# cristianpjensen/thesis-pai-reconstruction

Measured on AMD Instinct MI355X. Metric: train images/sec (256x256, bs=64) Pix2Pix step, higher is better.
Workload: dtype bf16; 1 GPU; Pix2Pix generator+PatchGAN GAN step, 256x256x1 pairs, 64 images/GPU (BASELINE configs[1]); global_batch=64, per_gpu_batch=64, loss_type=gan, parallelism=dp1, grad_bucket_dtype=f32

## Files before the change

### thesis-pai-reconstruction_amd/csrc/gg_thin.hip

```cpp
#include <stdlib.h>

#include "common.h"

#ifndef THIN_ABL
#define THIN_ABL 0
#endif
typedef __attribute__((ext_vector_type(8))) __bf16 bf8_t;
typedef __attribute__((ext_vector_type(4))) __bf16 bf4_t;
typedef __attribute__((ext_vector_type(4))) float f4_t;
typedef __attribute__((ext_vector_type(8))) short s8_t;
typedef __attribute__((ext_vector_type(8))) unsigned short us8_t;

__device__ uint4 g_zero_line_thin[16];


__device__ __forceinline__ bf8_t relu8(bf8_t f) {
    s8_t x = __builtin_bit_cast(s8_t, f);
    const s8_t z = {0, 0, 0, 0, 0, 0, 0, 0};
    return __builtin_bit_cast(bf8_t, __builtin_elementwise_max(x, z));
}

template <int S>
__device__ __forceinline__ us8_t thin_gather8(__amdgpu_buffer_rsrc_t rs, int e0, int ix0, int TW, bool valid) {
    typedef __attribute__((ext_vector_type(4))) unsigned u4_t;
    const int base = ix0 & ~1, o = ix0 & 1;
    const bool neg = valid && e0 + base < 0;
    const unsigned vo = valid ? (neg ? 0u : (unsigned)(e0 + base) * 2u) : 0x80000000u;
    unsigned out[4];
    if (S == 2) {
        u4_t a = __builtin_amdgcn_raw_buffer_load_b128(rs, (int)vo, 0, 0);
        u4_t b = __builtin_amdgcn_raw_buffer_load_b128(rs, (int)vo + 16, 0, 0);
        if (__builtin_amdgcn_ballot_w64(neg) != 0) {
            if (neg) { b = (u4_t){a[3], b[0], b[1], b[2]}; a = (u4_t){0u, a[0], a[1], a[2]}; }
        }
        const unsigned sel = o ? 0x07060302u : 0x05040100u;
        out[0] = __builtin_amdgcn_perm(a[1], a[0], sel);
        out[1] = __builtin_amdgcn_perm(a[3], a[2], sel);
        out[2] = __builtin_amdgcn_perm(b[1], b[0], sel);
        out[3] = __builtin_amdgcn_perm(b[3], b[2], sel);
    } else {
        u4_t a = __builtin_amdgcn_raw_buffer_load_b128(rs, (int)vo, 0, 0);
        unsigned a4 = __builtin_amdgcn_raw_buffer_load_b32(rs, (int)vo + 16, 0, 0);
        if (__builtin_amdgcn_ballot_w64(neg) != 0) {
            if (neg) { a4 = a[3]; a = (u4_t){0u, a[0], a[1], a[2]}; }
        }
        const unsigned sh = (unsigned)o * 16u;
        out[0] = __builtin_amdgcn_alignbit(a[1], a[0], sh);
        out[1] = __builtin_amdgcn_alignbit(a[2], a[1], sh);
        out[2] = __builtin_amdgcn_alignbit(a[3], a[2], sh);
        out[3] = __builtin_amdgcn_alignbit(a4, a[3], sh);
    }
    const bool edge = valid && (ix0 < 0 || ix0 + S * 7 >= TW);
    if (__builtin_amdgcn_ballot_w64(edge) != 0) {
// ... 160 lines not shown
    int p0 = (blockIdx.x * 4 + wid) * 16;
    us8_t pv = {0, 0, 0, 0, 0, 0, 0, 0};
    if (p0 < g.M) pv = fast ? gather_fast(p0) : gather(p0);
    for (; p0 < g.M; p0 += pstep) {
        const int m = p0 + fr;
        us8_t pnext = {0, 0, 0, 0, 0, 0, 0, 0};
        if (p0 + pstep < g.M) pnext = fast ? gather_fast(p0 + pstep) : gather(p0 + pstep);
        const bf8_t bfrag = __builtin_bit_cast(bf8_t, pv);
#pragma unroll
        for (int gq = 0; gq < 2; ++gq) {
            if (gq * 4 >= mtiles) break;
            float v[16];
#pragma unroll
            for (int q = 0; q < 4; ++q) {
                f4_t acc = {0.f, 0.f, 0.f, 0.f};
                acc = __builtin_amdgcn_mfma_f32_16x16x32_bf16(af[gq * 4 + q], bfrag, acc, 0, 0, 0);
#pragma unroll
                for (int r = 0; r < 4; ++r) v[4 * q + r] = acc[r] + bias[gq][4 * q + r];
            }
            if (m >= g.M) continue;
            if ((THIN_ABL & 2) && v[0] != 12345.f) continue;
            const int co = 64 * gq + (sect ? 8 : 16) * fq;
            const int hop = sect ? 32 : 8;
            const size_t pix = (size_t)m;
            if (a.y1 || a.y2) {
                unsigned pk[8];
#pragma unroll
                for (int e = 0; e < 8; ++e) pk[e] = pk2bf(v[2 * e], v[2 * e + 1]);
                bf16_t* dst = (co < g.D1) ? (bf16_t*)a.y1 + pix * g.D1 + co : (bf16_t*)a.y2 + pix * g.D2 + (co - g.D1);
                *(uint4*)dst = make_uint4(pk[0], pk[1], pk[2], pk[3]);
                *(uint4*)(dst + hop) = make_uint4(pk[4], pk[5], pk[6], pk[7]);
            }
            if (a.yact) {
                unsigned pk[8];
#pragma unroll
                for (int e = 0; e < 8; ++e) {
                    float v0 = fmaxf(v[2 * e], act_slope * v[2 * e]), v1 = fmaxf(v[2 * e + 1], act_slope * v[2 * e + 1]);
                    v0 = v0 < act_floor ? act_floor : v0;
                    v1 = v1 < act_floor ? act_floor : v1;
                    pk[e] = pk2bf(v0, v1);
                }
                bf16_t* dst = (bf16_t*)a.yact + pix * g.Cout + co;
                *(uint4*)dst = make_uint4(pk[0], pk[1], pk[2], pk[3]);
                *(uint4*)(dst + hop) = make_uint4(pk[4], pk[5], pk[6], pk[7]);
            }
        }
        pv = pnext;
    }
}

#ifndef THIN_BWD_WAVES
#define THIN_BWD_WAVES 1
#endif
template <int T, bool RAW, int ACTM, int NG, bool BWD = false>
__global__ __launch_bounds__(256, BWD ? THIN_BWD_WAVES : 1) void thin_fwd2_k(GG g, FwdArgs a) {
    const int tid = threadIdx.x, lane = tid & 63, wid = tid >> 6;
    const int fr = lane & 15, fq = lane >> 4;
    const bf16_t* w = (const bf16_t*)a.w;
    constexpr int mtiles = 4 * NG;
    constexpr int KT = 16 * T;
    bf8_t af[4 * NG];
#pragma unroll
    for (int mt = 0; mt < 4 * NG; ++mt) {
        us8_t z = {0, 0, 0, 0, 0, 0, 0, 0};
        const int co = 64 * (mt >> 2) + 32 * ((mt & 3) >> 1) + 8 * (fr >> 2) + 4 * (mt & 1) + (fr & 3);
        if (mt < mtiles && 8 * fq < KT) z = *(const us8_t*)(w + (size_t)co * KT + 8 * fq);
        af[mt] = __builtin_bit_cast(bf8_t, z);
    }
    f4_t bias4[NG][4];
#pragma unroll
    for (int gq = 0; gq < NG; ++gq)
#pragma unroll
        for (int q = 0; q < 4; ++q)
#pragma unroll
            for (int r = 0; r < 4; ++r)
                bias4[gq][q][r] = (!BWD && a.bias) ? a.bias[64 * gq + 32 * (q >> 1) + 8 * fq + 4 * (q & 1) + r] : 0.f;
    const int pdx0 = g.dx[0][(8 * fq < KT) ? (8 * fq) / T : 0];
    const int pdyA = g.dy[0][(8 * fq < KT) ? (8 * fq) / T : 0];
    const int pdyB = g.dy[0][(8 * fq + 4 < KT) ? (8 * fq + 4) / T : 0];
    const unsigned thin_bytes = (unsigned)(g.N * g.H * g.W) * 2u;
    const __amdgpu_buffer_rsrc_t rs1 = __builtin_amdgcn_make_buffer_rsrc(const_cast<void*>(a.x1), 0, thin_bytes, 0x00020000);
    const __amdgpu_buffer_rsrc_t rs2 = __builtin_amdgcn_make_buffer_rsrc(const_cast<void*>(T == 2 ? a.x2 : a.x1), 0, thin_bytes, 0x00020000);
    const bool lane_k = 8 * fq < KT;
    auto gather_fast = [&](int p0) {
        const int m = p0 + fr;
        int n, gy, gx;
        decode_row2(g, m < g.M ? m : 0, n, gy, gx);
        const int ix0 = gx * g.S + pdx0;
        const int iyA = gy * g.S + pdyA, iyB = gy * g.S + pdyB;
        const bool okA = lane_k && m < g.M && (unsigned)iyA < (unsigned)g.H;
        uint2 pa, pb;
        if (T == 1) {
            const bool okB = lane_k && m < g.M && (unsigned)iyB < (unsigned)g.H;
            pa = thin_gather4(rs1, (n * g.H + iyA) * g.W, ix0, g.W, okA);
            pb = thin_gather4(rs1, (n * g.H + iyB) * g.W, ix0, g.W, okB);
            if (g.relu1) { pa.x = relu2u(pa.x); pa.y = relu2u(pa.y); pb.x = relu2u(pb.x); pb.y = relu2u(pb.y); }
        } else {
            uint2 qa = thin_gather4(rs1, (n * g.H + iyA) * g.W, ix0, g.W, okA);
            uint2 qb = thin_gather4(rs2, (n * g.H + iyA) * g.W, ix0, g.W, okA);
            if (g.relu1) { qa.x = relu2u(qa.x); qa.y = relu2u(qa.y); }
            if (g.relu2) { qb.x = relu2u(qb.x); qb.y = relu2u(qb.y); }
            pa = make_uint2(__builtin_amdgcn_perm(qb.x, qa.x, 0x05040100u), __builtin_amdgcn_perm(qb.x, qa.x, 0x07060302u));
            pb = make_uint2(__builtin_amdgcn_perm(qb.y, qa.y, 0x05040100u), __builtin_amdgcn_perm(qb.y, qa.y, 0x07060302u));
        }
        return __builtin_bit_cast(us8_t, make_uint4(pa.x, pa.y, pb.x, pb.y));
    };
    const unsigned raw1_bytes = (unsigned)g.M * (unsigned)g.D1 * 2u, raw2_bytes = (unsigned)g.M * (unsigned)g.D2 * 2u;
    const __amdgpu_buffer_rsrc_t y1rs = __builtin_amdgcn_make_buffer_rsrc(a.y1, 0, RAW ? raw1_bytes : 0u, 0x00020000);
// ... 16 lines not shown
    us8_t pq[AHEAD];
#pragma unroll
    for (int i = 0; i < AHEAD; ++i) {
        pq[i] = (us8_t){0, 0, 0, 0, 0, 0, 0, 0};
        if ((int64_t)p0 + (int64_t)i * pstep < g.M) pq[i] = gather_fast(p0 + i * pstep);
    }
#ifndef THIN_ZA
#define THIN_ZA 2
#endif
    constexpr int ZA = THIN_ZA;
    u4_t zql[BWD ? ZA : 1], zqh[BWD ? ZA : 1];
    if (BWD) {
#pragma unroll
        for (int i = 0; i < ZA; ++i) {
            zql[i] = __builtin_amdgcn_raw_buffer_load_b128(zrs, (int)(o_r1 + (unsigned)i * s_r1), 0, 0);
            zqh[i] = __builtin_amdgcn_raw_buffer_load_b128(zrs, (int)(o_r1 + (unsigned)i * s_r1) + 64, 0, 0);
        }
    }
    for (; p0 < g.M; p0 += pstep) {
        us8_t pnext = {0, 0, 0, 0, 0, 0, 0, 0};
        if ((int64_t)p0 + (int64_t)AHEAD * pstep < g.M) pnext = gather_fast(p0 + AHEAD * pstep);
        const bf8_t bfrag = __builtin_bit_cast(bf8_t, pq[0]);
        u4_t zlo = {0u, 0u, 0u, 0u}, zhi = {0u, 0u, 0u, 0u};
        if (BWD) {
            zlo = zql[0]; zhi = zqh[0];
#pragma unroll
            for (int i = 0; i + 1 < ZA; ++i) { zql[i] = zql[i + 1]; zqh[i] = zqh[i + 1]; }
            const unsigned long long zo = (unsigned long long)o_r1 + (unsigned long long)ZA * s_r1;
            const int zoff = zo < (unsigned long long)raw1_bytes ? (int)(unsigned)zo : (int)0x80000000u;
            zql[ZA - 1] = __builtin_amdgcn_raw_buffer_load_b128(zrs, zoff, 0, 0);
            zqh[ZA - 1] = __builtin_amdgcn_raw_buffer_load_b128(zrs, zoff + 64, 0, 0);
        }
#pragma unroll
        for (int gq = 0; gq < NG; ++gq) {
            f4_t acc[4];
#pragma unroll
            for (int q = 0; q < 4; ++q) acc[q] = __builtin_amdgcn_mfma_f32_16x16x32_bf16(af[gq * 4 + q], bfrag, bias4[gq][q], 0, 0, 0);
            if (RAW) {
                const u4_t lo = {pk2bf(acc[0][0], acc[0][1]), pk2bf(acc[0][2], acc[0][3]), pk2bf(acc[1][0], acc[1][1]), pk2bf(acc[1][2], acc[1][3])};
                const u4_t hi = {pk2bf(acc[2][0], acc[2][1]), pk2bf(acc[2][2], acc[2][3]), pk2bf(acc[3][0], acc[3][1]), pk2bf(acc[3][2], acc[3][3])};
                if (BWD && gq == 0 && p0 + fr < g.M) {
#pragma unroll
                    for (int e = 0; e < 4; ++e) {
                        const float g0 = __uint_as_float(lo[e] << 16), g1 = __uint_as_float(lo[e] & 0xffff0000u);
                        const float h0 = __uint_as_float(hi[e] << 16), h1 = __uint_as_float(hi[e] & 0xffff0000u);
                        bs1[2 * e] += g0; bs1[2 * e + 1] += g1; bs1[8 + 2 * e] += h0; bs1[8 + 2 * e + 1] += h1;
                        bs2[2 * e] = fmaf(g0, __uint_as_float(zlo[e] << 16), bs2[2 * e]);
                        bs2[2 * e + 1] = fmaf(g1, __uint_as_float(zlo[e] & 0xffff0000u), bs2[2 * e + 1]);
                        bs2[8 + 2 * e] = fmaf(h0, __uint_as_float(zhi[e] << 16), bs2[8 + 2 * e]);
                        bs2[8 + 2 * e + 1] = fmaf(h1, __uint_as_float(zhi[e] & 0xffff0000u), bs2[8 + 2 * e + 1]);
                    }
                }
                if (gq == 1 && second_raw) {
                    __builtin_amdgcn_raw_buffer_store_b128(lo, y2rs, (int)o_r2, 0, 0);
                    __builtin_amdgcn_raw_buffer_store_b128(hi, y2rs, (int)o_r2 + 64, 0, 0);
                } else {
                    __builtin_amdgcn_raw_buffer_store_b128(lo, y1rs, (int)o_r1 + 128 * gq, 0, 0);
                    __builtin_amdgcn_raw_buffer_store_b128(hi, y1rs, (int)o_r1 + 128 * gq + 64, 0, 0);
                }
            }
            if (ACTM) {
#pragma unroll
                for (int q = 0; q < 4; ++q)
#pragma unroll
                    for (int r = 0; r < 4; ++r) {
                        if (ACTM == 1) acc[q][r] = fmaxf(acc[q][r], 0.2f * acc[q][r]);
                        else if (ACTM == 2) acc[q][r] = acc[q][r] < 0.f ? 0.f : acc[q][r];
                    }
                const u4_t lo = {pk2bf(acc[0][0], acc[0][1]), pk2bf(acc[0][2], acc[0][3]), pk2bf(acc[1][0], acc[1][1]), pk2bf(acc[1][2], acc[1][3])};
                const u4_t hi = {pk2bf(acc[2][0], acc[2][1]), pk2bf(acc[2][2], acc[2][3]), pk2bf(acc[3][0], acc[3][1]), pk2bf(acc[3][2], acc[3][3])};
                __builtin_amdgcn_raw_buffer_store_b128(lo, yars, (int)o_act + 128 * gq, 0, 0);
                __builtin_amdgcn_raw_buffer_store_b128(hi, yars, (int)o_act + 128 * gq + 64, 0, 0);
            }
        }
        o_act += s_act; o_r1 += s_r1; o_r2 += s_r2;
#pragma unroll
        for (int i = 0; i + 1 < AHEAD; ++i) pq[i] = pq[i + 1];
        pq[AHEAD - 1] = pnext;
    }
    if (BWD) {
        __shared__ float red[4][2][64];
#pragma unroll
        for (int c = 0; c < 16; ++c) {
            float s1 = bs1[c], s2 = bs2[c];
            s1 += __builtin_bit_cast(float, __builtin_amdgcn_update_dpp(0, __builtin_bit_cast(int, s1), 0xB1, 0xF, 0xF, false));
            s2 += __builtin_bit_cast(float, __builtin_amdgcn_update_dpp(0, __builtin_bit_cast(int, s2), 0xB1, 0xF, 0xF, false));
            s1 += __builtin_bit_cast(float, __builtin_amdgcn_update_dpp(0, __builtin_bit_cast(int, s1), 0x4E, 0xF, 0xF, false));
            s2 += __builtin_bit_cast(float, __builtin_amdgcn_update_dpp(0, __builtin_bit_cast(int, s2), 0x4E, 0xF, 0xF, false));
            s1 += __builtin_bit_cast(float, __builtin_amdgcn_update_dpp(0, __builtin_bit_cast(int, s1), 0x141, 0xF, 0xF, false));
            s2 += __builtin_bit_cast(float, __builtin_amdgcn_update_dpp(0, __builtin_bit_cast(int, s2), 0x141, 0xF, 0xF, false));
            s1 += __builtin_bit_cast(float, __builtin_amdgcn_update_dpp(0, __builtin_bit_cast(int, s1), 0x140, 0xF, 0xF, false));
            s2 += __builtin_bit_cast(float, __builtin_amdgcn_update_dpp(0, __builtin_bit_cast(int, s2), 0x140, 0xF, 0xF, false));
            if (fr == 0) {
                const int ch = (c < 8) ? 8 * fq + c : 32 + 8 * fq + (c - 8);
                red[wid][0][ch] = s1;
                red[wid][1][ch] = s2;
            }
        }
        __syncthreads();
        if (tid < 64) {
            const float s1 = red[0][0][tid] + red[1][0][tid] + red[2][0][tid] + red[3][0][tid];
            const float s2 = red[0][1][tid] + red[1][1][tid] + red[2][1][tid] + red[3][1][tid];
            float* row = a.bpart + (size_t)blockIdx.x * 2 * g.D1;
            row[tid] = s1;
            row[g.D1 + tid] = a.brstd[tid] * (s2 - a.bmean[tid] * s1);
        }
    }
}

template <int T>
static void launch_thin_fwd2(const GG& g, const FwdArgs& a, int blocks, hipStream_t s) {
    const bool raw = a.y1 || a.y2;
    const int actm = !a.yact ? 0 : (a.eact == PAI_ACT_LRELU ? 1 : (a.eact == PAI_ACT_RELU ? 2 : 3));
#define TF2(RAWV, ACTV)                                                                                   \
    do {                                                                                                  \
        if (g.Cout == 64) PAI_LAUNCH((thin_fwd2_k<T, RAWV, ACTV, 1>), dim3(blocks), dim3(256), 0, s, g, a); \
        else PAI_LAUNCH((thin_fwd2_k<T, RAWV, ACTV, 2>), dim3(blocks), dim3(256), 0, s, g, a);             \
    } while (0)
    if (raw && a.bz) {
        PAI_LAUNCH((thin_fwd2_k<1, true, 0, 2, true>), dim3(blocks), dim3(256), 0, s, g, a);
    } else if (raw) {
        if (actm == 0) TF2(true, 0); else if (actm == 1) TF2(true, 1); else if (actm == 2) TF2(true, 2); else TF2(true, 3);
    } else {
        if (actm == 1) TF2(false, 1); else if (actm == 2) TF2(false, 2); else TF2(false, 3);
    }
#undef TF2
}

static int thin_fwd_blocks(const GG& g) {
    int blocks = cdiv(g.M, 64);
    static const int cap = getenv("PAI_TF_BLOCKS") ? atoi(getenv("PAI_TF_BLOCKS")) : 4096;
    return blocks > cap ? cap : blocks;
}

static bool thin_fwd2_ok(const GG& g, const FwdArgs& a) {
    const bool fast = pai_tunable("thin_fast", 1) && (g.W % 2) == 0 && (int64_t)g.N * g.H * g.W * 2 < (1ll << 31) &&
                      pai_tunable("thin_sect", 1) && (g.D2 == 0 || (g.D1 % 64) == 0);
    const bool out_ok = (a.y1 || a.y2 || a.yact) && (!a.yact || a.eact != PAI_ACT_TANH) && (!a.y2 || a.y1) &&
                        (int64_t)g.M * g.Cout * 2 < (1ll << 32) && (g.D2 == 0 || (g.D1 == 64 && g.D2 == 64));
    return pai_tunable("thin_fwd2", 1) && fast && g.ntaps == 16 && out_ok && (g.Cout == 64 || g.Cout == 128) &&
           !(a.yact && (a.y1 || a.y2) && g.D2 > 0);
}

int thin_fwd_bwd_rows(int dtype, const GG& g, const FwdArgs& a, int act1, const void* add, const float* scale) {
    if (!thin_fwd_ok(dtype, g, a) || !thin_fwd2_ok(g, a) || !pai_tunable("thin_bwd", 1)) return 0;
    if (g.C2 != 0 || g.D1 != 64 || g.D2 != 64 || !a.y1 || !a.y2 || a.yact || act1 != PAI_ACT_NONE || add || scale) return 0;
    return thin_fwd_blocks(g);
}

int launch_thin_fwd(const GG& g, const FwdArgs& a, hipStream_t s) {
    int blocks = thin_fwd_blocks(g);
    int fast_ok = pai_tunable("thin_fast", 1) && (g.W % 2) == 0 && (int64_t)g.N * g.H * g.W * 2 < (1ll << 31);
    if (pai_tunable("thin_sect", 1) && (g.D2 == 0 || (g.D1 % 64) == 0)) fast_ok |= 2;
    if (thin_fwd2_ok(g, a)) {
        if (g.C2 == 0) launch_thin_fwd2<1>(g, a, blocks, s);
        else launch_thin_fwd2<2>(g, a, blocks, s);
        PAI_LAUNCH_CHECK();
        return 0;
    }
    if (g.C2 == 0) PAI_LAUNCH(thin_fwd_k<1>, dim3(blocks), dim3(256), 0, s, g, a, fast_ok);
    else PAI_LAUNCH(thin_fwd_k<2>, dim3(blocks), dim3(256), 0, s, g, a, fast_ok);
    PAI_LAUNCH_CHECK();
    return 0;
}

bool head_dgrad_ok(int dtype, const GG& g, const FwdArgs& a) {
    return dtype == PAI_BF16 && pai_tunable("head_dgrad", 1) && g.nphase == 1 && g.ntaps == 16 && g.S == 1 && g.OS == 1 &&
           g.C1 == 1 && g.C2 == 0 && g.D2 == 0 && g.Cout == g.D1 && (g.Cout % 8) == 0 && g.Cout <= 1024 && g.OW <= 64 &&
           g.H * g.W <= 4096 && a.y1 && !a.y2 && !a.yact && !a.yf32 && !a.stats && !a.bias && !g.relu1 && !a.badd &&
           !a.bscale && !a.bpart && !a.skip_d1;
}

__global__ __launch_bounds__(256) void head_dgrad_k(GG g, FwdArgs a) {
    extern __shared__ __attribute__((aligned(16))) unsigned char hsm[];
    bf16_t* wt = (bf16_t*)hsm;
    float* src = (float*)(hsm + (size_t)16 * g.Cout * 2);
    const int tid = threadIdx.x;
    const int n = blockIdx.x / g.OH, oy = blockIdx.x - n * g.OH;
    const bf16_t* w = (const bf16_t*)a.w;
    for (int i = tid; i < g.Cout * 16; i += 256) {
        const int c = i >> 4, t = i & 15;
        wt[t * g.Cout + c] = w[i];
    }
    const bf16_t* x = (const bf16_t*)a.x1 + (size_t)n * g.H * g.W;
// ... 260 lines not shown
        else if (T == 1) PAI_LAUNCH((thin_up_k<1, 2>), grid, dim3(256), 0, s, g, a, t0, tx, ty);
        else if (g.Cin == 128) PAI_LAUNCH((thin_up_k<2, 4>), grid, dim3(256), 0, s, g, a, t0, tx, ty);
        else PAI_LAUNCH((thin_up_k<2, 2>), grid, dim3(256), 0, s, g, a, t0, tx, ty);
        PAI_LAUNCH_CHECK();
        return 0;
    }
    int blocks = cdiv((int64_t)g.N * g.H * g.W, 256);
    if (blocks > 4096) blocks = 4096;
#define TDG(TT, KK) PAI_LAUNCH((thin_dgrad_gemm_k<TT, KK>), dim3(blocks), dim3(256), 0, s, g, a, pai_ctx()->scratch, t0)
#define TDG_K(TT)                                     \
    switch (g.Cin / 32) {                             \
        case 1: TDG(TT, 1); break;                    \
        case 2: TDG(TT, 2); break;                    \
        case 4: TDG(TT, 4); break;                    \
        case 8: TDG(TT, 8); break;                    \
        case 16: TDG(TT, 16); break;                  \
        default: PAI_CHECK(false, "thin dgrad: unsupported Cin %d", g.Cin); \
    }
    if (T == 1) { TDG_K(1) } else { TDG_K(2) }
#undef TDG_K
#undef TDG
    PAI_LAUNCH_CHECK();
    PAI_CHECK((int64_t)g.N * g.OH * g.OW < (1ll << 31), "thin dgrad: more than 2^31 output pixels");
    int64_t b2 = ((int64_t)g.N * g.OH * g.OW + 255) / 256;
    if (b2 > 8192) b2 = 8192;
    PAI_LAUNCH(thin_col2im_k, dim3((int)b2), dim3(256), 0, s, g, a, (const float*)pai_ctx()->scratch, T, t0);
    PAI_LAUNCH_CHECK();
    return 0;
}

struct ThinW {
    const bf16_t *thin1, *thin2;
    const bf16_t *wide1, *wide2;
    int N, H, W, TH, TW, WC1, WC2;
    int relu1, relu2;
    int lw, lh;
    int tmul, flip;
    int kw, ntaps;
    float* dw;
    int s_wc, s_tap, s_t;
    float* dbias;
    int M;
    int fast;
    int pair;
    float* partial;
};

__device__ __forceinline__ int tw_swz(int row) { return ((row & 3) << 2) | ((row >> 2) & 3); }
__device__ __forceinline__ unsigned tw_off(int row, int ch) { return (unsigned)(256 * row + 16 * (ch ^ tw_swz(row))); }

#ifndef THIN_WG_WAVES
#define THIN_WG_WAVES 1
#endif
template <int T>
__global__ __launch_bounds__(256, THIN_WG_WAVES) void thin_wgrad_k(ThinW p, int chunks_per_block) {
    extern __shared__ __attribute__((aligned(16))) unsigned char smem[];
    const int tid = threadIdx.x, lane = tid & 63;
    const int wid = __builtin_amdgcn_readfirstlane(tid >> 6);
    const int fr = lane & 15, fq = lane >> 4, tq = fr >> 2, tp = fr & 3;
    const int wc0 = blockIdx.y * 128;
    const int WC = min(p.WC1 + p.WC2 - wc0, 128);
    const int pair = p.pair;
    const int ntile = pair ? 8 : WC / 16;
    const int ks = wid & 1;
    const int nt0 = (wid >> 1) * (ntile / 2);
    const int ntn = ntile / 2;
    const int pixh = pair ? (wid >> 1) * 64 : 0;
    const int CH = pair ? 128 : 64;
    const bf16_t* zero = (const bf16_t*)g_zero_line_thin;

    const int sc = lane & 15, sr = wid * 4 + (lane >> 4);
    const int gch = sc ^ tw_swz(sr);
    const bf16_t* wsrc;
    int wstride, wcol;
    bool wvalid = pair || gch * 8 < WC;
    const int wpix = pair ? (gch >> 3) * 64 : 0;
    if (pair) { wsrc = p.wide1; wstride = p.WC1; wcol = (gch & 7) * 8; }
    else if (wc0 + gch * 8 < p.WC1) { wsrc = p.wide1; wstride = p.WC1; wcol = wc0 + gch * 8; }
    else { wsrc = p.wide2; wstride = p.WC2; wcol = gch * 8 - p.WC1; }

    int kdy[T], kdx[T];
    const bf16_t* ksrc[T];
    int kt[T];
#pragma unroll
    for (int tt = 0; tt < T; ++tt) {
        const int k = 16 * tt + fr;
        const int tap = k / T, t = k - tap * T;
        const int th = tap / p.kw, tw = tap - th * p.kw;
        kdy[tt] = p.flip ? 1 - th : th - 1;
        kdx[tt] = tap < p.ntaps ? (p.flip ? 1 - tw : tw - 1) : -(1 << 20);
        ksrc[tt] = t ? p.thin2 : p.thin1;
        kt[tt] = t;
    }
    const unsigned thin_bytes = (unsigned)(p.N * p.TH * p.TW) * 2u;
    const __amdgpu_buffer_rsrc_t trs1 = __builtin_amdgcn_make_buffer_rsrc(const_cast<bf16_t*>(p.thin1), 0, thin_bytes, 0x00020000);
    const __amdgpu_buffer_rsrc_t trs2 = __builtin_amdgcn_make_buffer_rsrc(
        const_cast<bf16_t*>(p.thin2 ? p.thin2 : p.thin1), 0, p.thin2 ? thin_bytes : 0u, 0x00020000);

    f4_t acc[T][4];
#pragma unroll
    for (int tt = 0; tt < T; ++tt)
#pragma unroll
        for (int j = 0; j < 4; ++j) acc[tt][j] = (f4_t){0.f, 0.f, 0.f, 0.f};
    f4_t accb[4];
#pragma unroll
    for (int j = 0; j < 4; ++j) accb[j] = (f4_t){0.f, 0.f, 0.f, 0.f};
    const unsigned one2 = fr == 0 ? 0x3f803f80u : 0u;
    const bf8_t ones = __builtin_bit_cast(bf8_t, make_uint4(one2, one2, one2, one2));

    for (int ci = 0; ci < chunks_per_block; ++ci) {
        const int p0 = (blockIdx.x * chunks_per_block + ci) * CH;
        if (p0 >= p.M) break;
#pragma unroll
        for (int j = 0; j < 4; ++j) {
            const int m = p0 + wpix + sr + 16 * j;
            const bf16_t* src = (wvalid && m < p.M) ? wsrc + (size_t)m * wstride + wcol : zero;
            __builtin_amdgcn_global_load_lds((const __attribute__((address_space(1))) void*)src,
                                             (__attribute__((address_space(3))) void*)(smem + (16 * j + wid * 4) * 256),
                                             16, 0, 0);
        }
        bf8_t af[T];
#pragma unroll
        for (int tt = 0; tt < T; ++tt) {
            us8_t pv;
            if (p.fast) {
                const int m = p0 + pixh + 32 * ks + 8 * fq;
                int n, ay, bx;
                if (p.lw >= 0) { bx = m & (p.W - 1); ay = (m >> p.lw) & (p.H - 1); n = m >> (p.lw + p.lh); }
                else { bx = m % p.W; const int r = m / p.W; ay = r % p.H; n = r / p.H; }
                const int iy = p.tmul * ay + kdy[tt], ix0 = p.tmul * bx + kdx[tt];
                const bool rowok = m < p.M && (unsigned)iy < (unsigned)p.TH && kdx[tt] > -(1 << 19);
                const int e0 = (n * p.TH + iy) * p.TW;
                if (p.tmul == 2) pv = kt[tt] ? thin_gather8<2>(trs2, e0, ix0, p.TW, rowok) : thin_gather8<2>(trs1, e0, ix0, p.TW, rowok);
                else pv = kt[tt] ? thin_gather8<1>(trs2, e0, ix0, p.TW, rowok) : thin_gather8<1>(trs1, e0, ix0, p.TW, rowok);
            } else {
#pragma unroll
            for (int j = 0; j < 8; ++j) {
                const int m = p0 + pixh + 32 * ks + 8 * fq + j;
                int n, ay, bx;
                if (p.lw >= 0) { bx = m & (p.W - 1); ay = (m >> p.lw) & (p.H - 1); n = m >> (p.lw + p.lh); }
                else { bx = m % p.W; const int r = m / p.W; ay = r % p.H; n = r / p.H; }
                const int iy = p.tmul * ay + kdy[tt], ix = p.tmul * bx + kdx[tt];
                const bool inb = m < p.M && (unsigned)iy < (unsigned)p.TH && (unsigned)ix < (unsigned)p.TW;
                pv[j] = inb ? ksrc[tt][(size_t)(n * p.TH + iy) * p.TW + ix] : (unsigned short)0;
            }
            }
            af[tt] = __builtin_bit_cast(bf8_t, pv);
        }
        __syncthreads();
#pragma unroll
        for (int nt = 0; nt < 4; ++nt) {
            if (nt >= ntn) break;
            const int col0 = (nt0 + nt) * 16;
            bf8_t bfr;
#pragma unroll
            for (int h = 0; h < 2; ++h) {
                const int row = ks * 32 + fq * 8 + h * 4 + tq;
                const int ch = col0 / 8 + (tp >> 1);
                bf4_t v = __builtin_amdgcn_ds_read_tr16_b64_v4bf16(
                    (bf4_t __attribute__((address_space(3)))*)(smem + tw_off(row, ch) + 8 * (tp & 1)));
#pragma unroll
                for (int e = 0; e < 4; ++e) bfr[h * 4 + e] = v[e];
// ... 66 lines not shown
        }
        for (; b < b1; b += 4) sum += src[(size_t)b * bstride];
    }
    red[slice][threadIdx.x & 63] = sum;
    __syncthreads();
    if (slice == 0 && gy < groups) {
        sum = red[0][threadIdx.x] + red[1][threadIdx.x] + red[2][threadIdx.x] + red[3][threadIdx.x];
        const int k = le >> 7;
        int wc = gy * 128 + (le & 127);
        if (p.pair) wc &= 63;
        if (wc < p.WC1 + p.WC2) {
            if (k < 16 * T) {
                const int tap = k / T, t = k - tap * T;
                if (tap < p.ntaps) atomicAdd(p.dw + (size_t)wc * p.s_wc + tap * p.s_tap + t * p.s_t, sum);
            } else if (p.dbias) {
                atomicAdd(p.dbias + wc, sum);
            }
        }
    }
}

__global__ __launch_bounds__(256) void sum1_k(const bf16_t* x, int64_t n, float* out) {
    __shared__ float ws[4];
    float s = 0.f;
    const int64_t n8 = n >> 3;
    for (int64_t i = (int64_t)blockIdx.x * 256 + threadIdx.x; i < n8; i += (int64_t)gridDim.x * 256) {
        const uint4 v = ((const uint4*)x)[i];
        const unsigned w4[4] = {v.x, v.y, v.z, v.w};
#pragma unroll
        for (int e = 0; e < 4; ++e) s += __uint_as_float(w4[e] << 16) + __uint_as_float(w4[e] & 0xffff0000u);
    }
    for (int64_t i = n8 * 8 + (int64_t)blockIdx.x * 256 + threadIdx.x; i < n; i += (int64_t)gridDim.x * 256) s += bf2f(x[i]);
    s = wave_sum(s);
    if ((threadIdx.x & 63) == 0) ws[threadIdx.x >> 6] = s;
    __syncthreads();
    if (threadIdx.x == 0) atomicAdd(out, ws[0] + ws[1] + ws[2] + ws[3]);
}

static int ilog2_exact(int v) {
    int l = 0;
    while ((1 << l) < v) ++l;
    return (1 << l) == v ? l : -1;
}

bool thin_wgrad_conv_ok(int dtype, const GG& g) {
    return dtype == PAI_BF16 && g.nphase == 1 && g.ntaps == 16 && g.S == 2 && g.OS == 1 && g.C1 == 1 &&
           g.C2 <= 1 && (g.Cout % 32) == 0 && g.Cout <= 128 && !g.relu1 && !g.relu2;
}
bool thin_wgrad_convt_ok(int dtype, const GG& g) {
    return dtype == PAI_BF16 && g.nphase == 4 && g.ntaps == 4 && g.Cout == 1 && (g.C1 % 8) == 0 &&
           (g.C2 % 8) == 0 && (g.Cin % 32) == 0 && g.Cin <= 128;
}

static int tw_blocks(int64_t M, int groups, bool two_stage) {
    static const int cap_env = getenv("PAI_TW_BLOCKS") ? atoi(getenv("PAI_TW_BLOCKS")) : 0;
    int cap = cap_env ? cap_env : (two_stage ? 1024 / groups : 512);
    if (cap < 64) cap = 64;
    const int chunks = cdiv(M, 64);
    int blocks = chunks < cap ? chunks : cap;
    const int cpb = cdiv(chunks, blocks);
    return cdiv(chunks, cpb);
}

int64_t thin_wgrad_scratch_bytes(int64_t M, int T, int WC) {
    return (int64_t)tw_blocks(M, cdiv(WC, 128), true) * 2 * cdiv(WC, 128) * (16 * T + 1) * 128 * sizeof(float);
}

static int launch_tw(ThinW& p, int T, hipStream_t s) {
    p.M = p.N * p.H * p.W;
    p.fast = pai_tunable("thin_fast", 1) && (p.W % 8) == 0 && (p.TW % 2) == 0 && (p.tmul == 1 || p.tmul == 2) &&
             (int64_t)p.N * p.TH * p.TW * 2 < (1ll << 31);
    p.lw = ilog2_exact(p.W);
    p.lh = ilog2_exact(p.H);
    if (p.lw < 0 || p.lh < 0) p.lw = p.lh = -1;
    p.pair = pai_tunable("thin_pair", 1) && p.WC1 == 64 && p.WC2 == 0 && T == 2;
    const int chunks = cdiv(p.M, p.pair ? 128 : 64);
    const int groups = cdiv(p.WC1 + p.WC2, 128);
    const int64_t need = thin_wgrad_scratch_bytes(p.M, T, p.WC1 + p.WC2);
    static const bool no_two = getenv("PAI_TW_ATOMIC") && atoi(getenv("PAI_TW_ATOMIC")) != 0;
    const pai_handle_s* ctx = pai_ctx();
    const bool two_stage = !no_two && ctx->scratch != nullptr && ctx->scratch_bytes >= need;
    int blocks = tw_blocks(p.M, groups, two_stage);
    const int cpb = cdiv(chunks, blocks);
    p.partial = two_stage ? (float*)((char*)ctx->scratch + (ctx->scratch_bytes - need)) : nullptr;
    if (T == 1) PAI_LAUNCH(thin_wgrad_k<1>, dim3(blocks, groups), dim3(256), 64 * 256, s, p, cpb);
    else PAI_LAUNCH(thin_wgrad_k<2>, dim3(blocks, groups), dim3(256), 64 * 256, s, p, cpb);
    PAI_LAUNCH_CHECK();
    if (two_stage) {
        const int elems = groups * (16 * T + 1) * 128;
        PAI_LAUNCH(thin_wgrad_reduce_k, dim3(cdiv(elems, 64), 16), dim3(256), 0, s, p, T, blocks * 2, groups);
        PAI_LAUNCH_CHECK();
    }
    return 0;
}

int launch_thin_wgrad_conv(const GG& g, const WgradArgs& a, hipStream_t s) {
    ThinW p;
    memset(&p, 0, sizeof(p));
    const int T = g.C1 + g.C2;
    p.thin1 = (const bf16_t*)a.x1; p.thin2 = (const bf16_t*)a.x2;
    p.wide1 = (const bf16_t*)a.dy; p.wide2 = nullptr;
    p.N = g.N; p.H = g.OHg; p.W = g.OWg; p.TH = g.H; p.TW = g.W;
    p.WC1 = g.Cout; p.WC2 = 0;
    p.dw = a.dw; p.s_wc = 16 * T; p.s_tap = T; p.s_t = 1;
    p.dbias = a.dbias;
    p.tmul = 2; p.flip = 0; p.kw = 4; p.ntaps = 16;
    return launch_tw(p, T, s);
}

int launch_thin_wgrad_convt(const GG& g, const WgradArgs& a, hipStream_t s) {
    ThinW p;
    memset(&p, 0, sizeof(p));
    p.thin1 = (const bf16_t*)a.dy; p.thin2 = nullptr;
    p.wide1 = (const bf16_t*)a.x1; p.wide2 = (const bf16_t*)a.x2;
    p.N = g.N; p.H = g.H; p.W = g.W; p.TH = g.OH; p.TW = g.OW;
    p.WC1 = g.C1; p.WC2 = g.C2; p.relu1 = g.relu1; p.relu2 = g.relu2;
    p.dw = a.dw; p.s_wc = 1; p.s_tap = g.Cin; p.s_t = 0;
    p.dbias = nullptr;
    p.tmul = 2; p.flip = 0; p.kw = 4; p.ntaps = 16;
    if (launch_tw(p, 1, s)) return 1;
    if (a.dbias) {
        const int64_t n = (int64_t)g.N * g.OH * g.OW;
        PAI_LAUNCH(sum1_k, dim3(256), dim3(256), 0, s, (const bf16_t*)a.dy, n, a.dbias);
        PAI_LAUNCH_CHECK();
    }
    return 0;
}

bool thin_wgrad_conv1_ok(int dtype, const GG& g) {
    return dtype == PAI_BF16 && g.nphase == 1 && g.ntaps == 16 && g.S == 1 && g.OS == 1 && g.Cout == 1 &&
           g.C2 == 0 && (g.C1 % 128) == 0;
}

int launch_thin_wgrad_conv1(const GG& g, const WgradArgs& a, hipStream_t s) {
    ThinW p;
    memset(&p, 0, sizeof(p));
    p.thin1 = (const bf16_t*)a.dy; p.thin2 = nullptr;
    p.wide1 = (const bf16_t*)a.x1; p.wide2 = nullptr;
// ... 56 lines not shown
```

Measured before the change: 11260 images/s.

## Add three-stage LDS ring pipeline to thin wgrad and nontemporal fwd stores

```diff
diff --git a/thesis-pai-reconstruction_amd/csrc/gg_thin.hip b/thesis-pai-reconstruction_amd/csrc/gg_thin.hip
--- a/thesis-pai-reconstruction_amd/csrc/gg_thin.hip
+++ b/thesis-pai-reconstruction_amd/csrc/gg_thin.hip
@@ -1,4 +1,6 @@
 #include <stdlib.h>
+
+#include <type_traits>
 
 #include "common.h"
 
@@ -265,8 +267,9 @@
 #ifndef THIN_BWD_WAVES
 #define THIN_BWD_WAVES 1
 #endif
-template <int T, bool RAW, int ACTM, int NG, bool BWD = false>
+template <int T, bool RAW, int ACTM, int NG, bool BWD = false, bool NT = false>
 __global__ __launch_bounds__(256, BWD ? THIN_BWD_WAVES : 1) void thin_fwd2_k(GG g, FwdArgs a) {
+    constexpr int SAUX = NT ? 2 : 0;
     const int tid = threadIdx.x, lane = tid & 63, wid = tid >> 6;
     const int fr = lane & 15, fq = lane >> 4;
     const bf16_t* w = (const bf16_t*)a.w;
@@ -389,11 +392,11 @@
                     }
                 }
                 if (gq == 1 && second_raw) {
-                    __builtin_amdgcn_raw_buffer_store_b128(lo, y2rs, (int)o_r2, 0, 0);
-                    __builtin_amdgcn_raw_buffer_store_b128(hi, y2rs, (int)o_r2 + 64, 0, 0);
+                    __builtin_amdgcn_raw_buffer_store_b128(lo, y2rs, (int)o_r2, 0, SAUX);
+                    __builtin_amdgcn_raw_buffer_store_b128(hi, y2rs, (int)o_r2 + 64, 0, SAUX);
                 } else {
-                    __builtin_amdgcn_raw_buffer_store_b128(lo, y1rs, (int)o_r1 + 128 * gq, 0, 0);
-                    __builtin_amdgcn_raw_buffer_store_b128(hi, y1rs, (int)o_r1 + 128 * gq + 64, 0, 0);
+                    __builtin_amdgcn_raw_buffer_store_b128(lo, y1rs, (int)o_r1 + 128 * gq, 0, SAUX);
+                    __builtin_amdgcn_raw_buffer_store_b128(hi, y1rs, (int)o_r1 + 128 * gq + 64, 0, SAUX);
                 }
             }
             if (ACTM) {
@@ -406,8 +409,8 @@
                     }
                 const u4_t lo = {pk2bf(acc[0][0], acc[0][1]), pk2bf(acc[0][2], acc[0][3]), pk2bf(acc[1][0], acc[1][1]), pk2bf(acc[1][2], acc[1][3])};
                 const u4_t hi = {pk2bf(acc[2][0], acc[2][1]), pk2bf(acc[2][2], acc[2][3]), pk2bf(acc[3][0], acc[3][1]), pk2bf(acc[3][2], acc[3][3])};
-                __builtin_amdgcn_raw_buffer_store_b128(lo, yars, (int)o_act + 128 * gq, 0, 0);
-                __builtin_amdgcn_raw_buffer_store_b128(hi, yars, (int)o_act + 128 * gq + 64, 0, 0);
+                __builtin_amdgcn_raw_buffer_store_b128(lo, yars, (int)o_act + 128 * gq, 0, SAUX);
+                __builtin_amdgcn_raw_buffer_store_b128(hi, yars, (int)o_act + 128 * gq + 64, 0, SAUX);
             }
         }
         o_act += s_act; o_r1 += s_r1; o_r2 += s_r2;
@@ -445,28 +448,45 @@
     }
 }
 
+#ifndef THIN_FWD_NT_MB
+#define THIN_FWD_NT_MB 128
+#endif
+static bool thin_fwd_nt(const GG& g) {
+    const int64_t bytes = (int64_t)g.M * (g.D2 > 0 ? g.D1 : g.Cout) * 2;
+    return bytes >= (int64_t)pai_tunable("thin_fwd_nt_mb", THIN_FWD_NT_MB) << 20;
+}
+
 template <int T>
 static void launch_thin_fwd2(const GG& g, const FwdArgs& a, int blocks, hipStream_t s) {
     const bool raw = a.y1 || a.y2;
+    const bool nt = thin_fwd_nt(g);
     const int actm = !a.yact ? 0 : (a.eact == PAI_ACT_LRELU ? 1 : (a.eact == PAI_ACT_RELU ? 2 : 3));
-#define TF2(RAWV, ACTV)                                                                                   \
-    do {                                                                                                  \
-        if (g.Cout == 64) PAI_LAUNCH((thin_fwd2_k<T, RAWV, ACTV, 1>), dim3(blocks), dim3(256), 0, s, g, a); \
-        else PAI_LAUNCH((thin_fwd2_k<T, RAWV, ACTV, 2>), dim3(blocks), dim3(256), 0, s, g, a);             \
+#define TF2N(RAWV, ACTV, NTV)                                                                                           \
+    do {                                                                                                                \
+        if (g.Cout == 64) PAI_LAUNCH((thin_fwd2_k<T, RAWV, ACTV, 1, false, NTV>), dim3(blocks), dim3(256), 0, s, g, a); \
+        else PAI_LAUNCH((thin_fwd2_k<T, RAWV, ACTV, 2, false, NTV>), dim3(blocks), dim3(256), 0, s, g, a);             \
+    } while (0)
+#define TF2(RAWV, ACTV)                                            \
+    do {                                                           \
+        if (nt) TF2N(RAWV, ACTV, true); else TF2N(RAWV, ACTV, false); \
     } while (0)
     if (raw && a.bz) {
-        PAI_LAUNCH((thin_fwd2_k<1, true, 0, 2, true>), dim3(blocks), dim3(256), 0, s, g, a);
+        if (nt) PAI_LAUNCH((thin_fwd2_k<1, true, 0, 2, true, true>), dim3(blocks), dim3(256), 0, s, g, a);
+        else PAI_LAUNCH((thin_fwd2_k<1, true, 0, 2, true>), dim3(blocks), dim3(256), 0, s, g, a);
     } else if (raw) {
         if (actm == 0) TF2(true, 0); else if (actm == 1) TF2(true, 1); else if (actm == 2) TF2(true, 2); else TF2(true, 3);
     } else {
         if (actm == 1) TF2(false, 1); else if (actm == 2) TF2(false, 2); else TF2(false, 3);
     }
 #undef TF2
+#undef TF2N
 }
 
 static int thin_fwd_blocks(const GG& g) {
     int blocks = cdiv(g.M, 64);
-    static const int cap = getenv("PAI_TF_BLOCKS") ? atoi(getenv("PAI_TF_BLOCKS")) : 4096;
+    static const int cap_env = getenv("PAI_TF_BLOCKS") ? atoi(getenv("PAI_TF_BLOCKS")) : 4096;
+    const int cap_tun = pai_tunable("thin_fwd_blocks", 0);
+    const int cap = cap_tun > 0 ? cap_tun : cap_env;
     return blocks > cap ? cap : blocks;
 }
 
@@ -833,8 +853,44 @@
 #ifndef THIN_WG_WAVES
 #define THIN_WG_WAVES 1
 #endif
-template <int T>
-__global__ __launch_bounds__(256, THIN_WG_WAVES) void thin_wgrad_k(ThinW p, int chunks_per_block) {
+typedef __attribute__((ext_vector_type(4))) unsigned tw_u4_t;
+typedef __attribute__((ext_vector_type(4))) int tw_i4_t;
+__device__ __forceinline__ void tw_load32(tw_u4_t& a, tw_u4_t& b, unsigned vo, tw_i4_t rs) {
+    asm volatile("buffer_load_dwordx4 %[a], %[vo], %[rs], 0 offen\n\tbuffer_load_dwordx4 %[b], %[vo], %[rs], 0 offen offset:16"
+                 : [a] "=&v"(a), [b] "=&v"(b) : [vo] "v"(vo), [rs] "s"(rs) : "memory");
+}
+__device__ __forceinline__ void tw_load32x2(tw_u4_t& a, tw_u4_t& b, unsigned vo, tw_i4_t rs1, tw_i4_t rs2) {
+    unsigned long long sv;
+    asm volatile("s_mov_b64 %[sv], exec\n\t"
+                 "s_and_b64 exec, %[sv], %[even]\n\t"
+                 "buffer_load_dwordx4 %[a], %[vo], %[r1], 0 offen\n\t"
+                 "buffer_load_dwordx4 %[b], %[vo], %[r1], 0 offen offset:16\n\t"
+                 "s_andn2_b64 exec, %[sv], %[even]\n\t"
+                 "buffer_load_dwordx4 %[a], %[vo], %[r2], 0 offen\n\t"
+                 "buffer_load_dwordx4 %[b], %[vo], %[r2], 0 offen offset:16\n\t"
+                 "s_mov_b64 exec, %[sv]"
+                 : [a] "=&v"(a), [b] "=&v"(b), [sv] "=&s"(sv)
+                 : [vo] "v"(vo), [r1] "s"(rs1), [r2] "s"(rs2), [even] "s"(0x5555555555555555ull) : "memory", "scc");
+}
+typedef __attribute__((ext_vector_type(2))) unsigned tw_u2_t;
+template <int OFF>
+__device__ __forceinline__ void tw_read_tr2(tw_u2_t& lo, tw_u2_t& hi, unsigned a0, unsigned a1) {
+    asm volatile("ds_read_b64_tr_b16 %0, %2 offset:%4\n\tds_read_b64_tr_b16 %1, %3 offset:%4"
+                 : "=&v"(lo), "=&v"(hi) : "v"(a0), "v"(a1), "n"(OFF) : "memory");
+}
+template <int T, int N>
+__device__ __forceinline__ void tw_retire(tw_u4_t (&ga)[T], tw_u4_t (&gb)[T]) {
+    if constexpr (T == 2)
+        asm volatile("s_waitcnt vmcnt(%[n])" : "+v"(ga[0]), "+v"(gb[0]), "+v"(ga[1]), "+v"(gb[1]) : [n] "n"(N) : "memory");
+    else
+        asm volatile("s_waitcnt vmcnt(%[n])" : "+v"(ga[0]), "+v"(gb[0]) : [n] "n"(N) : "memory");
+}
+
+#ifndef THIN_WG_RING_WAVES
+#define THIN_WG_RING_WAVES 3
+#endif
+template <int T, int S = 1>
+__global__ __launch_bounds__(256, S > 1 ? THIN_WG_RING_WAVES : THIN_WG_WAVES) void thin_wgrad_k(ThinW p, int chunks_per_block) {
     extern __shared__ __attribute__((aligned(16))) unsigned char smem[];
     const int tid = threadIdx.x, lane = tid & 63;
     const int wid = __builtin_amdgcn_readfirstlane(tid >> 6);
@@ -889,6 +945,117 @@
     const unsigned one2 = fr == 0 ? 0x3f803f80u : 0u;
     const bf8_t ones = __builtin_bit_cast(bf8_t, make_uint4(one2, one2, one2, one2));
 
+    if constexpr (S > 1) {
+        static_assert(S == 3, "the loop below is unrolled for a ring of three");
+        constexpr int LG = T == 2 ? 8 : 2;
+        constexpr int LT = 4;
+        const int c_first = blockIdx.x * chunks_per_block;
+        const int nchunk = min(chunks_per_block, (p.M + CH - 1) / CH - c_first);
+        const unsigned long long a1 = (unsigned long long)p.thin1, a2 = (unsigned long long)(p.thin2 ? p.thin2 : p.thin1);
+        const tw_i4_t ars1 = {(int)(unsigned)a1, (int)((unsigned)(a1 >> 32) & 0xffffu), (int)thin_bytes, 0x00020000};
+        const tw_i4_t ars2 = {(int)(unsigned)a2, (int)((unsigned)(a2 >> 32) & 0xffffu), (int)(p.thin2 ? thin_bytes : 0u), 0x00020000};
+        auto geom = [&](int c, int tt, int& e0, int& ix0, bool& rowok) {
+            const int m = (c_first + c) * CH + pixh + 32 * ks + 8 * fq;
+            int n, ay, bx;
+            if (p.lw >= 0) { bx = m & (p.W - 1); ay = (m >> p.lw) & (p.H - 1); n = m >> (p.lw + p.lh); }
+            else { bx = m % p.W; const int r = m / p.W; ay = r % p.H; n = r / p.H; }
+            const int iy = p.tmul * ay + kdy[tt];
+            ix0 = p.tmul * bx + kdx[tt];
+            rowok = c < nchunk && m < p.M && (unsigned)iy < (unsigned)p.TH && kdx[tt] > -(1 << 19);
+            e0 = (n * p.TH + iy) * p.TW;
+        };
+        unsigned long long wsrc_v = (unsigned long long)wsrc;
+        auto issue = [&](int c, unsigned char* st, tw_u4_t (&ga)[T], tw_u4_t (&gb)[T]) {
+#pragma unroll
+            for (int tt = 0; tt < T; ++tt) {
+                int e0, ix0;
+                bool rowok;
+                geom(c, tt, e0, ix0, rowok);
+                const int base = ix0 & ~1;
+                const bool neg = rowok && e0 + base < 0;
+                const unsigned vo = rowok ? (neg ? 0u : (unsigned)(e0 + base) * 2u) : 0x80000000u;
+                if constexpr (T == 2) tw_load32x2(ga[tt], gb[tt], vo, ars1, ars2);
+                else tw_load32(ga[tt], gb[tt], vo, ars1);
+            }
+            const int p0 = (c_first + c) * CH;
+            const bool live = c < nchunk;
+#pragma unroll
+            for (int j = 0; j < 4; ++j) {
+                const int m = p0 + wpix + sr + 16 * j;
+                const bf16_t* src = (live && wvalid && m < p.M) ? (const bf16_t*)wsrc_v + (size_t)m * wstride + wcol : zero;
+                __builtin_amdgcn_global_load_lds((const __attribute__((address_space(1))) void*)src,
+                                                 (__attribute__((address_space(3))) void*)(st + (16 * j + wid * 4) * 256),
+                                                 16, 0, 0);
+            }
+        };
+        auto finish = [&](int c, int tt, tw_u4_t a, tw_u4_t b) {
+            int e0, ix0;
+            bool rowok;
+            geom(c, tt, e0, ix0, rowok);
+            const int base = ix0 & ~1, o = ix0 & 1;
+            const bool neg = rowok && e0 + base < 0;
+            if (__builtin_amdgcn_ballot_w64(neg) != 0) {
+                if (neg) { b = (tw_u4_t){a[3], b[0], b[1], b[2]}; a = (tw_u4_t){0u, a[0], a[1], a[2]}; }
+            }
+            const unsigned sel = o ? 0x07060302u : 0x05040100u;
+            unsigned out[4] = {__builtin_amdgcn_perm(a[1], a[0], sel), __builtin_amdgcn_perm(a[3], a[2], sel),
+                               __builtin_amdgcn_perm(b[1], b[0], sel), __builtin_amdgcn_perm(b[3], b[2], sel)};
+            const bool edge = rowok && (ix0 < 0 || ix0 + 14 >= p.TW);
+            if (__builtin_amdgcn_ballot_w64(edge) != 0) {
+#pragma unroll
+                for (int i = 0; i < 4; ++i) {
+                    const bool lo = (unsigned)(ix0 + 4 * i) < (unsigned)p.TW, hi = (unsigned)(ix0 + 4 * i + 2) < (unsigned)p.TW;
+                    out[i] &= (lo ? 0xffffu : 0u) | (hi ? 0xffff0000u : 0u);
+                }
+            }
+            return __builtin_bit_cast(bf8_t, make_uint4(out[0], out[1], out[2], out[3]));
+        };
+        const unsigned lds0 = (unsigned)(size_t)(__attribute__((address_space(3))) unsigned char*)smem;
+        tw_u4_t ga[3][T], gb[3][T];
+        asm volatile("" : "+v"(wsrc_v));
+        issue(0, smem, ga[0], gb[0]);
+        issue(1, smem + 16384, ga[1], gb[1]);
+        auto step = [&](auto k_tag, int c) {
+            constexpr int k = decltype(k_tag)::value;
+            {
+                tw_retire<T, LG + LT>(ga[k], gb[k]);
+                __builtin_amdgcn_s_barrier();
+                issue(c + 2, smem + ((k + 2) % 3) * 16384, ga[(k + 2) % 3], gb[(k + 2) % 3]);
+                tw_u2_t flo[4], fhi[4];
+#pragma unroll
+                for (int nt = 0; nt < 4; ++nt) {
+                    if (nt >= ntn) break;
+                    const int ch = (nt0 + nt) * 2 + (tp >> 1);
+                    const int row = ks * 32 + fq * 8 + tq;
+                    tw_read_tr2<k * 16384>(flo[nt], fhi[nt], lds0 + tw_off(row, ch) + 8 * (tp & 1), lds0 + tw_off(row + 4, ch) + 8 * (tp & 1));
+                }
+                bf8_t af[T];
+#pragma unroll
+                for (int tt = 0; tt < T; ++tt) af[tt] = finish(c, tt, ga[k][tt], gb[k][tt]);
+                asm volatile("s_waitcnt lgkmcnt(0)" ::: "memory");
+#pragma unroll
+                for (int nt = 0; nt < 4; ++nt) {
+                    if (nt >= ntn) break;
+                    asm volatile("" : "+v"(flo[nt]), "+v"(fhi[nt]));
+                    const int col0 = (nt0 + nt) * 16;
+                    bf8_t bfr = __builtin_bit_cast(bf8_t, make_uint4(flo[nt].x, flo[nt].y, fhi[nt].x, fhi[nt].y));
+                    if ((pair || wc0 + col0 < p.WC1) ? p.relu1 : p.relu2) bfr = relu8(bfr);
+#pragma unroll
+                    for (int tt = 0; tt < T; ++tt)
+                        acc[tt][nt] = __builtin_amdgcn_mfma_f32_16x16x32_bf16(af[tt], bfr, acc[tt][nt], 0, 0, 0);
+                    if (p.dbias) accb[nt] = __builtin_amdgcn_mfma_f32_16x16x32_bf16(ones, bfr, accb[nt], 0, 0, 0);
+                }
+            }
+        };
+        for (int c = 0; c < nchunk; c += 3) {
+            step(std::integral_constant<int, 0>{}, c);
+            if (c + 1 >= nchunk) break;
+            step(std::integral_constant<int, 1>{}, c + 1);
+            if (c + 2 >= nchunk) break;
+            step(std::integral_constant<int, 2>{}, c + 2);
+        }
+        asm volatile("s_waitcnt vmcnt(0)" ::: "memory");
+    } else
     for (int ci = 0; ci < chunks_per_block; ++ci) {
         const int p0 = (blockIdx.x * chunks_per_block + ci) * CH;
         if (p0 >= p.M) break;
@@ -1061,10 +1228,12 @@
            (g.C2 % 8) == 0 && (g.Cin % 32) == 0 && g.Cin <= 128;
 }
 
-static int tw_blocks(int64_t M, int groups, bool two_stage) {
+static int tw_blocks(int64_t M, int groups, bool two_stage, int per_cu = 4) {
     static const int cap_env = getenv("PAI_TW_BLOCKS") ? atoi(getenv("PAI_TW_BLOCKS")) : 0;
-    int cap = cap_env ? cap_env : (two_stage ? 1024 / groups : 512);
+    int cap = cap_env ? cap_env : (two_stage ? 256 * per_cu / groups : 512);
     if (cap < 64) cap = 64;
+    const int cap_tun = pai_tunable("thin_wgrad_blocks", 0);
+    if (cap_tun > 0) cap = cap_tun;
     const int chunks = cdiv(M, 64);
     int blocks = chunks < cap ? chunks : cap;
     const int cpb = cdiv(chunks, blocks);
@@ -1075,6 +1244,9 @@
     return (int64_t)tw_blocks(M, cdiv(WC, 128), true) * 2 * cdiv(WC, 128) * (16 * T + 1) * 128 * sizeof(float);
 }
 
+#ifndef THIN_WG_STAGES_DEFAULT
+#define THIN_WG_STAGES_DEFAULT 3
+#endif
 static int launch_tw(ThinW& p, int T, hipStream_t s) {
     p.M = p.N * p.H * p.W;
     p.fast = pai_tunable("thin_fast", 1) && (p.W % 8) == 0 && (p.TW % 2) == 0 && (p.tmul == 1 || p.tmul == 2) &&
@@ -1089,10 +1261,14 @@
     static const bool no_two = getenv("PAI_TW_ATOMIC") && atoi(getenv("PAI_TW_ATOMIC")) != 0;
     const pai_handle_s* ctx = pai_ctx();
     const bool two_stage = !no_two && ctx->scratch != nullptr && ctx->scratch_bytes >= need;
-    int blocks = tw_blocks(p.M, groups, two_stage);
+    const bool ring = pai_tunable("thin_wgrad_stages", THIN_WG_STAGES_DEFAULT) >= 3 && p.fast && p.tmul == 2;
+    int blocks = tw_blocks(p.M, groups, two_stage, ring ? min(max(pai_tunable("thin_wgrad_ring_wgs", 3), 1), 4) : 4);
     const int cpb = cdiv(chunks, blocks);
     p.partial = two_stage ? (float*)((char*)ctx->scratch + (ctx->scratch_bytes - need)) : nullptr;
-    if (T == 1) PAI_LAUNCH(thin_wgrad_k<1>, dim3(blocks, groups), dim3(256), 64 * 256, s, p, cpb);
+    if (ring) {
+        if (T == 1) PAI_LAUNCH((thin_wgrad_k<1, 3>), dim3(blocks, groups), dim3(256), 3 * 64 * 256, s, p, cpb);
+        else PAI_LAUNCH((thin_wgrad_k<2, 3>), dim3(blocks, groups), dim3(256), 3 * 64 * 256, s, p, cpb);
+    } else if (T == 1) PAI_LAUNCH(thin_wgrad_k<1>, dim3(blocks, groups), dim3(256), 64 * 256, s, p, cpb);
     else PAI_LAUNCH(thin_wgrad_k<2>, dim3(blocks, groups), dim3(256), 64 * 256, s, p, cpb);
     PAI_LAUNCH_CHECK();
     if (two_stage) {
```

Measured after the change: 11220 images/s. Within noise of the previous version (-0.3%).
